# JCBrouwer/maua-style

Measured on AMD Instinct MI355X. Metric: optimizer iterations/sec at 1024x1024 VGG-19, higher is better.
Workload: dtype f32 (fp16x3 split-precision MFMA, fp32 accumulate)

## Files before the change

maua-style_amd/csrc/conv_x3w.hip:

```cpp
#include <stdlib.h>

#include <type_traits>

#include "conv_host.hpp"
#include "fp16x3.hpp"

namespace maua {

constexpr int XW_COT = 64;
constexpr int XW_ROWS = 8, XW_PR = 10, XW_PC = 34;
constexpr int XW_NPOS = XW_PR * XW_PC;
constexpr int XW_NPOS_PAD = 344;
constexpr int XW_PLANE = XW_NPOS_PAD * 16;
constexpr int XW_PATCH_BYTES = 4 * XW_PLANE;
constexpr int XW_W_BYTES = 9 * 2 * 2 * XW_COT * 16;
constexpr int XW_ITEMS = 2 * XW_NPOS;

__global__ void pack_x3w_kernel(const float* __restrict__ w, unsigned short* __restrict__ bank, int cout, int cin, int backward,
                                float w_scale) {
    const int CO = backward ? cin : cout;
    const int CI = backward ? cout : cin;
    const int nchunk = (CI + 15) / 16, ntile = (CO + XW_COT - 1) / XW_COT;
    const int64_t total = (int64_t)nchunk * ntile * 9 * 2 * XW_COT * 8;
    for (int64_t e = (int64_t)blockIdx.x * blockDim.x + threadIdx.x; e < total; e += (int64_t)gridDim.x * blockDim.x) {
        int64_t r = e;
        const int ch = (int)(r % 8);
        r /= 8;
        const int co = (int)(r % XW_COT);
        r /= XW_COT;
        const int oct = (int)(r % 2);
        r /= 2;
        const int tap = (int)(r % 9);
        r /= 9;
        const int tile = (int)(r % ntile);
        const int chunk = (int)(r / ntile);
        const int o = tile * XW_COT + co, i = chunk * 16 + oct * 8 + ch;
        float v = 0.f;
        if (o < CO && i < CI) {
            if (!backward) v = w[((int64_t)o * cin + i) * 9 + tap];
            else v = w[((int64_t)i * cin + o) * 9 + (8 - tap)];
        }
        v *= w_scale;
        const _Float16 h = (_Float16)v;
        const _Float16 l = (_Float16)(v - (float)h);
        const int64_t base = ((int64_t)chunk * ntile + tile) * (XW_W_BYTES / 2);
        bank[base + ((((int64_t)tap * 2 + 0) * 2 + oct) * XW_COT + co) * 8 + ch] = __builtin_bit_cast(unsigned short, h);
        bank[base + ((((int64_t)tap * 2 + 1) * 2 + oct) * XW_COT + co) * 8 + ch] = __builtin_bit_cast(unsigned short, l);
    }
}

__device__ __forceinline__ void pack_dmat_x3w_body(const float* __restrict__ d, int C, unsigned short* __restrict__ bank,
                                                   float* __restrict__ inv) {
    __shared__ float wmax[16];
    const int tid = threadIdx.x;
    const int64_t total4 = (int64_t)C * C / 4;
    float m = 0.f;
    int64_t e = tid;
    for (; e + 7 * 1024 < total4; e += 8 * 1024) {
        float4 v[8];
#pragma unroll
        for (int u = 0; u < 8; ++u) v[u] = reinterpret_cast<const float4*>(d)[e + u * 1024];
#pragma unroll
        for (int u = 0; u < 8; ++u) m = fmaxf(fmaxf(m, fmaxf(fabsf(v[u].x), fabsf(v[u].y))), fmaxf(fabsf(v[u].z), fabsf(v[u].w)));
    }
    for (; e < total4; e += 1024) {
        const float4 v = reinterpret_cast<const float4*>(d)[e];
        m = fmaxf(fmaxf(m, fmaxf(fabsf(v.x), fabsf(v.y))), fmaxf(fabsf(v.z), fabsf(v.w)));
    }
    m = wave_max_nonneg(m);
    if ((tid & 63) == 0) wmax[tid >> 6] = m;
    __syncthreads();
    m = 0.f;
    for (int i = 0; i < 16; ++i) m = fmaxf(m, wmax[i]);
    float scale = 1.f;
    if (m > 0.f && m < 3.0e38f) {
        const int e = (int)((__builtin_bit_cast(unsigned, m) >> 23) & 0xffu) - 127;
        scale = __builtin_bit_cast(float, (unsigned)(127 + 5 - max(e, -100)) << 23);
    }
    if (tid == 0 && blockIdx.x == 0) inv[0] = 1.f / scale;
    const int nchunk = C / 16, ntile = (C + XW_COT - 1) / XW_COT;
    const int64_t groups = (int64_t)nchunk * ntile * 2 * XW_COT;
    for (int64_t e = (int64_t)blockIdx.x * 1024 + tid; e < groups; e += (int64_t)gridDim.x * 1024) {
        int64_t r = e;
        const int co = (int)(r % XW_COT);
        r /= XW_COT;
        const int oct = (int)(r % 2);
        r /= 2;
        const int tile = (int)(r % ntile);
        const int chunk = (int)(r / ntile);
        const int o = tile * XW_COT + co, i = chunk * 16 + oct * 8;
        u32x4 Hh = {0u, 0u, 0u, 0u}, Ll = {0u, 0u, 0u, 0u};
        if (o < C) {
            const float4 v0 = *reinterpret_cast<const float4*>(d + (int64_t)o * C + i);
            const float4 v1 = *reinterpret_cast<const float4*>(d + (int64_t)o * C + i + 4);
            const float v[8] = {v0.x * scale, v0.y * scale, v0.z * scale, v0.w * scale, v1.x * scale, v1.y * scale, v1.z * scale, v1.w * scale};
#pragma unroll
            for (int q = 0; q < 4; ++q) {
                const unsigned H = cvt_pk_f16(v[2 * q], v[2 * q + 1]);
                Hh[q] = H;
                Ll[q] = cvt_pk_f16(v[2 * q] - f16_lo(H), v[2 * q + 1] - f16_hi(H));
            }
        }
        unsigned char* base = reinterpret_cast<unsigned char*>(bank) + ((int64_t)chunk * ntile + tile) * 4096 + co * 16;
        *reinterpret_cast<u32x4*>(base + (0 * 2 + oct) * 1024) = Hh;
        *reinterpret_cast<u32x4*>(base + (1 * 2 + oct) * 1024) = Ll;
    }
}
__global__ void __launch_bounds__(1024) pack_dmat_x3w_kernel(const float* __restrict__ d, int C, unsigned short* __restrict__ bank,
                                                             float* __restrict__ inv) {
    pack_dmat_x3w_body(d, C, bank, inv);
}
struct DmatPackBatch {
    const float* d[4];
    unsigned short* bank[4];
    float* inv[4];
    int C[4];
};
__global__ void __launch_bounds__(1024) pack_dmat_x3w_batch_kernel(DmatPackBatch b) {
    pack_dmat_x3w_body(b.d[blockIdx.y], b.C[blockIdx.y], b.bank[blockIdx.y], b.inv[blockIdx.y]);
}

#ifdef XW_STAMP
#define XW_MARK(k)                                                                                          \
    do {                                                                                                    \
        if (lane == 0 && p.mask) {                                                                          \
            const unsigned long long t_ = __builtin_amdgcn_s_memtime();                                     \
            const_cast<float*>(p.mask)[((((int64_t)blockIdx.y * gridDim.x + blockIdx.x) * 4 + wave) * 64 + (ch - ch_begin)) * 8 + (k)] = \
                __builtin_bit_cast(float, (unsigned)t_);                                                    \
        }                                                                                                   \
    } while (0)
#else
#define XW_MARK(k) do {} while (0)
#endif
#ifdef XW_STAMP
#define XW_END_STAMP()                                                                                      \
    do {                                      \
        asm volatile("s_waitcnt vmcnt(0)" ::: "memory");                                                    \
        if (lane == 0 && p.mask)                                                                            \
            const_cast<float*>(p.mask)[((((int64_t)blockIdx.y * gridDim.x + blockIdx.x) * 4 + wave) * 64 + 63) * 8 + 6] = \
                __builtin_bit_cast(float, (unsigned)__builtin_amdgcn_s_memtime());                          \
    } while (0)
#else
#define XW_END_STAMP() do {} while (0)
#endif

__device__ __forceinline__ const ConvArgs* xw_kernel_arguments() {
#if defined(__HIP_DEVICE_COMPILE__)
    return (const ConvArgs*)__builtin_amdgcn_kernarg_segment_ptr();
#else
    return nullptr;
#endif
}

template <bool ACC, bool OM, bool POOL = false, bool UNPOOL = false>
__global__ void __launch_bounds__(256, 2) conv_x3w_kernel(ConvArgs p, float w_inv_scale) {
    __shared__ __attribute__((aligned(16))) unsigned char smem[XW_PATCH_BYTES + XW_W_BYTES + 32];
    unsigned char* Pl = smem;
    unsigned char* Wl = smem + XW_PATCH_BYTES;
    float* Ml = reinterpret_cast<float*>(smem + XW_PATCH_BYTES + XW_W_BYTES);

    const int tid = threadIdx.x;
    const int lane = tid & 63, wave = tid >> 6;
    const int j = lane & 31, half = lane >> 5;
    const int wv = __builtin_amdgcn_readfirstlane(wave);
    const int ksplit = p.ksplit > 1 ? p.ksplit : 1;
    const int n = blockIdx.z / ksplit, split = blockIdx.z - n * ksplit;
    const int ntile = gridDim.y;
    const int tiles_total = p.tiles_x * ((p.OH + XW_ROWS - 1) / XW_ROWS);
    const int per_xcd = (tiles_total + 7) >> 3;
    const int xcd = blockIdx.x & 7;
    const int slot = (int)((blockIdx.y * gridDim.x + blockIdx.x) >> 3);
    const int cotile = p.cot_inner ? slot % ntile : (int)blockIdx.y;
    const int tile = xcd * per_xcd + (p.cot_inner ? slot / ntile : (int)(blockIdx.x >> 3));
    const int co0 = cotile * XW_COT;
    const int in_plane = p.H * p.W;
    const int64_t out_plane = (int64_t)p.OH * p.OW;
    const int st_w = UNPOOL ? p.W >> 1 : p.W;
    const int st_plane = UNPOOL ? (p.H >> 1) * (p.W >> 1) : in_plane;
    const float* __restrict__ xin = p.x + (int64_t)n * p.Cin * st_plane;
    const unsigned char* __restrict__ xcodes = UNPOOL ? p.in_codes + (int64_t)n * p.Cin * st_plane : nullptr;
    const unsigned code_mask = (unsigned)p.in_code_mask;
    if (tile >= min((xcd + 1) * per_xcd, tiles_total)) return;
    const int x0 = (tile % p.tiles_x) * 32, y0 = (tile / p.tiles_x) * XW_ROWS;
    if (tid == 0) {
        reinterpret_cast<int*>(Ml)[5] = (n * ntile + cotile) * tiles_total + tile;
        reinterpret_cast<int*>(Ml)[6] = split;
    }

    unsigned voff[3], lds_w[3];
    unsigned vcode = 0x80000000u, inmask = 0;
    if constexpr (UNPOOL) {
        constexpr int PR = XW_ROWS / 2 + 2, PCW = 18;
        const int oct = tid >= PR * PCW ? 1 : 0;
        const int rem = tid - oct * PR * PCW;
        const int pr = rem / PCW, pc = rem - pr * PCW;
        const int ppy = ((y0 - p.pad) >> 1) + pr, ppx = ((x0 - p.pad) >> 1) + pc;
        const bool item = tid < 2 * PR * PCW;
        const bool ok = item && ppy >= 0 && ppy < (p.H >> 1) && ppx >= 0 && ppx < st_w;
        const int pidx = ppy * st_w + ppx;
        voff[0] = ok ? (unsigned)(oct * 8 * st_plane + pidx) * 4u : 0x80000000u;
        vcode = ok ? (unsigned)(oct * st_plane + pidx) * 8u : 0x80000000u;
        const int r0 = 2 * ppy - (y0 - p.pad), c0 = 2 * ppx - (x0 - p.pad);
#pragma unroll
        for (int q = 0; q < 4; ++q) {
            const int r = r0 + (q >> 1), c = c0 + (q & 1);
            if (item && r >= 0 && r < XW_ROWS + 2 && c >= 0 && c < XW_PC) inmask |= 1u << q;
        }
        lds_w[0] = (unsigned)(oct * XW_PLANE + (r0 * XW_PC + c0) * 16);
        voff[1] = voff[2] = 0x80000000u;
        lds_w[1] = lds_w[2] = 0;
    } else {
#pragma unroll
        for (int k = 0; k < 3; ++k) {
            const int idx = tid + 256 * k;
            const int oct = idx >= XW_NPOS ? 1 : 0;
            const int pos = idx - oct * XW_NPOS;
            const int r = pos / XW_PC, c = pos - r * XW_PC;
            const int iy = y0 + r - p.pad, ix = x0 + c - p.pad;
            const bool ok = idx < XW_ITEMS && iy >= 0 && iy < p.H && ix >= 0 && ix < p.W;
            voff[k] = ok ? (unsigned)(oct * 8 * in_plane + iy * p.W + ix) * 4u : 0x80000000u;
            lds_w[k] = (unsigned)(oct * XW_PLANE + pos * 16);
        }
    }
    const unsigned range = (unsigned)in_plane * 64u;
    const unsigned range_x = (unsigned)st_plane * 64u;
    constexpr int NI = UNPOOL ? 1 : 3;
    float rp[NI][8];
    u32x2 cd = {0u, 0u};
    unsigned sel2[4];
    u32x4 hl[3][2];
    const int nmain = p.Cin / 16;
    const int n2 = p.dbank ? p.Cout / 16 : 0;
    const float* __restrict__ fin = p.dbank ? p.omask + (int64_t)n * p.Cout * in_plane : nullptr;
    auto load_patch = [&](int ch) {
        asm volatile("" : "+s"(ch));
        const __amdgpu_buffer_rsrc_t rs = __builtin_amdgcn_make_buffer_rsrc(const_cast<float*>(xin + (int64_t)ch * 16 * st_plane), 0, range_x, 0x00020000);
        if constexpr (UNPOOL) {
            const __amdgpu_buffer_rsrc_t rc = __builtin_amdgcn_make_buffer_rsrc(const_cast<unsigned char*>(xcodes + (int64_t)ch * 16 * st_plane), 0,
                                                                                range_x >> 2, 0x00020000);
            cd = __builtin_amdgcn_raw_buffer_load_b64(rc, vcode, 0, 0);
        }
#pragma unroll
        for (int c = 0; c < 8; ++c)
#pragma unroll
            for (int k = 0; k < NI; ++k)
                rp[k][c] = __builtin_bit_cast(float, __builtin_amdgcn_raw_buffer_load_b32(rs, voff[k], c * st_plane * 4, 0));
    };
    auto publish_max = [&]() {
        if constexpr (UNPOOL) {
            const unsigned m2 = code_mask * 0x00010001u;
#pragma unroll
            for (int i = 0; i < 4; ++i) {
                sel2[i] = __builtin_amdgcn_perm(0u, cd[i >> 1], (i & 1) ? 0x0c030c02u : 0x0c010c00u) & m2;
                const unsigned s0 = sel2[i] & 0xffffu, s1 = sel2[i] >> 16;
                rp[0][2 * i] = ((inmask >> s0) & 1u) ? rp[0][2 * i] : 0.f;
                rp[0][2 * i + 1] = ((inmask >> s1) & 1u) ? rp[0][2 * i + 1] : 0.f;
            }
        }
        float m = 0.f;
#pragma unroll
        for (int k = 0; k < NI; ++k)
#pragma unroll
            for (int c = 0; c < 8; ++c) m = fmaxf(m, fabsf(rp[k][c]));
        m = wave_max_nonneg(m);
        if (lane == 0) Ml[UNPOOL ? wv : wave] = m;
    };
    float sx = 1.f;
    auto chunk_scale = [&]() {
        const float m = fmaxf(fmaxf(Ml[0], Ml[1]), fmaxf(Ml[2], Ml[3]));
        int e = (int)((__builtin_bit_cast(unsigned, m) >> 23) & 0xffu) - 127;
        e = m > 0.f ? max(e, -100) : 11;
        sx = __builtin_bit_cast(float, (unsigned)(127 + 11 - e) << 23);
        return __builtin_bit_cast(float, (unsigned)(127 + e - 11) << 23);
    };
    auto corner_of = [&](int q, int part, int i) {
        const unsigned t = sel2[i] ^ ((unsigned)q * 0x00010001u);
        const unsigned keep = ((t & 0xffffu) ? 0u : 0xffffu) | ((t >> 16) ? 0u : 0xffff0000u);
        return hl[2][part][i] & keep;
    };
    auto split_item = [&](int k) {
        if constexpr (UNPOOL) {
            if (k == 1) {
#pragma unroll
                for (int q = 0; q < 2; ++q)
#pragma unroll
                    for (int i = 0; i < 4; ++i) {
                        hl[q][0][i] = corner_of(q, 0, i);
                        hl[q][1][i] = corner_of(q, 1, i);
                    }
            }
            if (k > 0) return;
        }
        const int dst = UNPOOL ? 2 : k;
#pragma unroll
        for (int q = 0; q < 4; ++q) {
            const float v0 = rp[k][2 * q] * sx, v1 = rp[k][2 * q + 1] * sx;
            const unsigned H = cvt_pk_f16(v0, v1);
            const unsigned Lo = cvt_pk_f16(v0 - f16_lo(H), v1 - f16_hi(H));
            hl[dst][0][q] = H;
            hl[dst][1][q] = Lo;
        }
    };
    auto store_patch = [&]() {
        if constexpr (UNPOOL) {
#pragma unroll
            for (int q = 0; q < 4; ++q)
                if ((inmask >> q) & 1u) {
                    const unsigned dst = lds_w[0] + (unsigned)(((q >> 1) * XW_PC + (q & 1)) * 16);
                    u32x4 h, l;
                    if (q < 2) {
                        h = hl[q][0];
                        l = hl[q][1];
                    } else {
#pragma unroll
                        for (int i = 0; i < 4; ++i) {
                            h[i] = corner_of(q, 0, i);
                            l[i] = corner_of(q, 1, i);
                        }
                    }
                    *reinterpret_cast<u32x4*>(Pl + dst) = h;
                    *reinterpret_cast<u32x4*>(Pl + 2 * XW_PLANE + dst) = l;
                }
            return;
        }
#pragma unroll
        for (int k = 0; k < NI; ++k) {
            if (k == 2 && tid >= XW_ITEMS - 512) break;
            *reinterpret_cast<u32x4*>(Pl + lds_w[k]) = hl[k][0];
            *reinterpret_cast<u32x4*>(Pl + 2 * XW_PLANE + lds_w[k]) = hl[k][1];
        }
    };

    const unsigned char* __restrict__ bank = reinterpret_cast<const unsigned char*>(p.w6);
    const unsigned lane16 = lane * 16;
    auto dma_filters = [&](int ch, int first, int count) {
        const unsigned char* src = bank + ((int64_t)ch * ntile + cotile) * XW_W_BYTES;
#pragma unroll
        for (int i = 0; i < count; ++i) {
            const int q = first + wv + 4 * i;
            const unsigned char* g = src + q * 1024;
            const unsigned lds_dst = (unsigned)(size_t)(__attribute__((address_space(3))) unsigned char*)(Wl + q * 1024);
            unsigned keep;
            asm volatile("s_mov_b32 %0, m0\n\ts_mov_b32 m0, %2\n\ts_nop 0\n\tglobal_load_lds_dwordx4 %1, %3\n\ts_mov_b32 m0, %0"
                         : "=&s"(keep)
                         : "v"(lane16), "s"(__builtin_amdgcn_readfirstlane(lds_dst)), "s"(g)
                         : "memory");
        }
    };

    const unsigned char* __restrict__ dbank = reinterpret_cast<const unsigned char*>(p.dbank);
    const float d_inv_scale = p.dbank ? p.dinv[n] : 0.f;

    const int b_base = half * XW_PLANE + ((2 * wave) * XW_PC + j) * 16;
    const int a_base = half * 1024 + j * 16;

    f32x16 acc[2][2], master[2][2];
    {
        const bool with_bias = p.bias != nullptr && p.ksplit <= 1;
#pragma unroll
        for (int t = 0; t < 2; ++t)
#pragma unroll
            for (int r = 0; r < 16; ++r) {
                const int co = co0 + t * 32 + (r & 3) + 8 * (r >> 2) + 4 * half;
                float b0 = 0.f;
                if (with_bias) b0 = p.bias[min(co, p.Cout - 1)];
                master[t][0][r] = b0;
                master[t][1][r] = b0;
                acc[t][0][r] = 0.f;
                acc[t][1][r] = 0.f;
            }
    }

    typedef f16x8 AFrag[2];
    typedef f16x8 BFrag[2][2];
    auto load_a = [&](AFrag& a, int tap, int t) {
#pragma unroll
        for (int part = 0; part < 2; ++part)
            a[part] = *reinterpret_cast<const f16x8*>(Wl + a_base + (tap * 2 + part) * 2048 + t * 512);
    };
    auto load_b = [&](BFrag& b, int tap) {
        const int ky = tap / 3, kx = tap - 3 * ky;
#pragma unroll
        for (int row = 0; row < 2; ++row)
#pragma unroll
            for (int part = 0; part < 2; ++part)
                b[row][part] = *reinterpret_cast<const f16x8*>(Pl + b_base + part * 2 * XW_PLANE + ((row + ky) * XW_PC + kx) * 16);
    };
    auto mfma_half = [&](const AFrag& a, const BFrag& b, int t) {
#pragma unroll
        for (int row = 0; row < 2; ++row) {
            acc[t][row] = __builtin_amdgcn_mfma_f32_32x32x16_f16(a[1], b[row][0], acc[t][row], 0, 0, 0);
            acc[t][row] = __builtin_amdgcn_mfma_f32_32x32x16_f16(a[0], b[row][1], acc[t][row], 0, 0, 0);
            acc[t][row] = __builtin_amdgcn_mfma_f32_32x32x16_f16(a[0], b[row][0], acc[t][row], 0, 0, 0);
        }
    };
    AFrag a0, a1;
    BFrag bx, by;
#define XW_FENCE() __builtin_amdgcn_sched_barrier(0)
#define XW_TAP(TAP, BCUR, BNXT, HAS_NEXT, EXTRA0, EXTRA1) \
    do {                                                  \
        load_a(a1, TAP, 1);                               \
        if (HAS_NEXT) load_b(BNXT, (TAP) + 1);            \
        XW_FENCE();                                       \
        mfma_half(a0, BCUR, 0);                           \
        EXTRA0;                                           \
        XW_FENCE();                                       \
        if (HAS_NEXT) load_a(a0, (TAP) + 1, 0);           \
        XW_FENCE();                                       \
        mfma_half(a1, BCUR, 1);                           \
        EXTRA1;                                           \
        XW_FENCE();                                       \
    } while (0)

    const int nchunks_all = nmain + n2;
    const int cps = (nchunks_all + ksplit - 1) / ksplit;
    const int ch_begin = split * cps;
    const int nchunks = min(nchunks_all, ch_begin + cps);
    float inv_cur = 0.f, inv_next = 0.f;
    if (ch_begin < min(nchunks, nmain)) {
        dma_filters(ch_begin, 0, 9);
        load_patch(ch_begin);
        publish_max();
        asm volatile("s_waitcnt lgkmcnt(0)" ::: "memory");
        __builtin_amdgcn_s_barrier();
        inv_cur = chunk_scale() * w_inv_scale;
        inv_next = inv_cur;
#pragma unroll
        for (int k = 0; k < 3; ++k) split_item(k);
        store_patch();
        asm volatile("s_waitcnt vmcnt(0) lgkmcnt(0)" ::: "memory");
        __builtin_amdgcn_s_barrier();
    }

    if (p.stagger > 0) {
        const int tg_slot = (__builtin_amdgcn_s_getreg((4 - 1) << 11 | 16 << 6 | 4) & 1);
        const int flat = blockIdx.x + gridDim.x * (blockIdx.y + gridDim.y * blockIdx.z);
        if (tg_slot && flat < 512)
            for (int i = 0; i < p.stagger; ++i) __builtin_amdgcn_s_sleep(8);
    }

#ifdef XW_STAMP
    if (lane == 0 && p.mask) {
        float* d_ = const_cast<float*>(p.mask) + ((((int64_t)blockIdx.y * gridDim.x + blockIdx.x) * 4 + wave) * 64 + 63) * 8;
        d_[0] = __builtin_bit_cast(float, (unsigned)__builtin_amdgcn_s_getreg((32 - 1) << 11 | 0 << 6 | 4));
        d_[1] = __builtin_bit_cast(float, (unsigned)__builtin_amdgcn_s_memtime());
        d_[2] = __builtin_bit_cast(float, (unsigned)__builtin_amdgcn_s_memrealtime());
    }
#endif
    const int main_end = min(nchunks, nmain);
    const int d_begin = max(ch_begin, nmain);
    for (int ch = ch_begin; ch < main_end; ++ch) {
        const bool more = ch + 1 < main_end;
        XW_MARK(0);
        load_b(bx, 0);
        load_a(a0, 0, 0);
        if (more) load_patch(ch + 1);
        XW_FENCE();
        XW_TAP(0, bx, by, true, (void)0, (void)0);
        XW_TAP(1, by, bx, true, (void)0, (void)0);
        XW_TAP(2, bx, by, true, (void)0, (void)0);
        XW_TAP(3, by, bx, true, (void)0, (void)0);
        XW_TAP(4, bx, by, true, (void)0, if (more) publish_max());
        XW_MARK(1);
        asm volatile("s_waitcnt lgkmcnt(0)" ::: "memory");
        XW_MARK(2);
        __builtin_amdgcn_s_barrier();
        XW_MARK(3);
        if (more) {
            dma_filters(ch + 1, 0, 5);
            inv_next = chunk_scale() * w_inv_scale;
        }
        XW_FENCE();
        XW_TAP(5, by, bx, true, if (more) split_item(0), (void)0);
        XW_TAP(6, bx, by, true, if (more) split_item(1), (void)0);
        XW_TAP(7, by, bx, true, if (more) split_item(2), (void)0);
        XW_TAP(8, bx, by, false, (void)0, (void)0);
        XW_MARK(4);
        asm volatile("s_waitcnt lgkmcnt(0)" ::: "memory");
        __builtin_amdgcn_s_barrier();
        XW_MARK(5);
        if (more) {
            dma_filters(ch + 1, 20, 4);
            store_patch();
        }
#pragma unroll
        for (int t = 0; t < 2; ++t)
#pragma unroll
            for (int row = 0; row < 2; ++row)
#pragma unroll
                for (int r = 0; r < 16; ++r) {
                    master[t][row][r] = fmaf(acc[t][row][r], inv_cur, master[t][row][r]);
                    acc[t][row][r] = 0.f;
                }
        inv_cur = inv_next;
        XW_MARK(6);
        if (more) {
            asm volatile("s_waitcnt vmcnt(0) lgkmcnt(0)" ::: "memory");
            XW_MARK(7);
            __builtin_amdgcn_s_barrier();
        }
    }

#ifdef XW_STAMP
    if (lane == 0 && p.mask) {
        float* d_ = const_cast<float*>(p.mask) + ((((int64_t)blockIdx.y * gridDim.x + blockIdx.x) * 4 + wave) * 64 + 63) * 8;
        d_[5] = __builtin_bit_cast(float, (unsigned)__builtin_amdgcn_s_memtime());
    }
#endif
    [[maybe_unused]] unsigned fbits[2] = {0u, 0u};
    [[maybe_unused]] const bool mask_from_bits = OM && p.mask_bits != 0;
    if constexpr (!POOL) if (d_begin < nchunks) {
        unsigned voff_f[2];
#pragma unroll
        for (int row = 0; row < 2; ++row) {
            const int oy = y0 + 2 * wave + row, oxx = x0 + j;
            voff_f[row] = (oy < p.H && oxx < p.W) ? (unsigned)(half * 8 * in_plane + oy * p.W + oxx) * 4u : 0x80000000u;
        }
        struct DChunk {
            float f[2][8];
            u32x4 a[2][2];
        };
        auto request = [&](DChunk& d, int c2) {
            asm volatile("" : "+s"(c2));
            const __amdgpu_buffer_rsrc_t rs = __builtin_amdgcn_make_buffer_rsrc(const_cast<float*>(fin + (int64_t)c2 * 16 * in_plane), 0, range, 0x00020000);
#pragma unroll
            for (int c = 0; c < 8; ++c)
#pragma unroll
                for (int row = 0; row < 2; ++row)
                    d.f[row][c] = __builtin_bit_cast(float, __builtin_amdgcn_raw_buffer_load_b32(rs, voff_f[row], c * in_plane * 4, 0));
            const unsigned char* g = dbank + (((int64_t)n * n2 + c2) * ntile + cotile) * 4096 + half * 1024 + j * 16;
#pragma unroll
            for (int part = 0; part < 2; ++part)
#pragma unroll
                for (int t = 0; t < 2; ++t) d.a[part][t] = *reinterpret_cast<const u32x4*>(g + part * 2048 + t * 512);
        };
        const int c2_begin = d_begin - nmain, c2_end = nchunks - nmain;
        DChunk da, db;
        request(da, c2_begin);
        __builtin_amdgcn_s_barrier();
        auto multiply = [&](DChunk& d, int c2) {
            if constexpr (OM) {
                const unsigned k = (unsigned)(c2 - (co0 >> 4));
                if (mask_from_bits && k < 4u) {
#pragma unroll
                    for (int row = 0; row < 2; ++row) {
                        unsigned b8 = 0;
#pragma unroll
                        for (int c = 0; c < 8; ++c) b8 |= d.f[row][c] > 0.f ? 1u << c : 0u;
                        fbits[row] |= b8 << (8 * k);
                    }
                }
            }
            float m = 0.f;
#pragma unroll
            for (int row = 0; row < 2; ++row)
#pragma unroll
                for (int c = 0; c < 8; ++c) m = fmaxf(m, fabsf(d.f[row][c]));
            m = wave_max_nonneg(m);
            int e = (int)((__builtin_bit_cast(unsigned, m) >> 23) & 0xffu) - 127;
            e = m > 0.f ? max(e, -100) : 11;
            const float s = __builtin_bit_cast(float, (unsigned)(127 + 11 - e) << 23);
            const float inv = __builtin_bit_cast(float, (unsigned)(127 + e - 11) << 23) * d_inv_scale;
            BFrag b;
#pragma unroll
            for (int row = 0; row < 2; ++row) {
                u32x4 Hh, Ll;
#pragma unroll
                for (int q = 0; q < 4; ++q) {
                    const float v0 = d.f[row][2 * q] * s, v1 = d.f[row][2 * q + 1] * s;
                    const unsigned H = cvt_pk_f16(v0, v1);
                    Hh[q] = H;
                    Ll[q] = cvt_pk_f16(v0 - f16_lo(H), v1 - f16_hi(H));
                }
                b[row][0] = __builtin_bit_cast(f16x8, Hh);
                b[row][1] = __builtin_bit_cast(f16x8, Ll);
            }
#pragma unroll
            for (int t = 0; t < 2; ++t) {
                AFrag a;
                a[0] = __builtin_bit_cast(f16x8, d.a[0][t]);
                a[1] = __builtin_bit_cast(f16x8, d.a[1][t]);
                mfma_half(a, b, t);
            }
#pragma unroll
            for (int t = 0; t < 2; ++t)
#pragma unroll
                for (int row = 0; row < 2; ++row)
#pragma unroll
                    for (int q = 0; q < 16; ++q) {
                        master[t][row][q] = fmaf(acc[t][row][q], inv, master[t][row][q]);
                        acc[t][row][q] = 0.f;
                    }
        };
        for (int c2 = c2_begin; c2 < c2_end; c2 += 2) {
            if (c2 + 1 < c2_end) request(db, c2 + 1);
            multiply(da, c2);
            if (c2 + 1 < c2_end) {
                if (c2 + 2 < c2_end) request(da, c2 + 2);
                multiply(db, c2 + 1);
            }
        }
    }

#ifdef XW_STAMP
    if (lane == 0 && p.mask) {
        float* d_ = const_cast<float*>(p.mask) + ((((int64_t)blockIdx.y * gridDim.x + blockIdx.x) * 4 + wave) * 64 + 63) * 8;
        d_[3] = __builtin_bit_cast(float, (unsigned)__builtin_amdgcn_s_memtime());
        d_[4] = __builtin_bit_cast(float, (unsigned)__builtin_amdgcn_s_memrealtime());
    }
#endif
    bool final_sums = p.ksplit <= 1;
    const ConvArgs* kp = xw_kernel_arguments();
    asm volatile("" : "+s"(kp));
    if (kp->ksplit > 1 && kp->arrive != nullptr) {
        const int ksplit = kp->ksplit;
        const int unit = __builtin_amdgcn_readfirstlane(reinterpret_cast<const int*>(Ml)[5]);
        const int split = __builtin_amdgcn_readfirstlane(reinterpret_cast<const int*>(Ml)[6]);
        unsigned* const arrive = kp->arrive + unit;
        const float* const bias = kp->bias;
        constexpr unsigned SLAB = XW_COT * XW_ROWS * 32 * 4;
        const __amdgpu_buffer_rsrc_t srs = __builtin_amdgcn_make_buffer_rsrc(reinterpret_cast<unsigned char*>(kp->ws) + (int64_t)unit * ksplit * SLAB, 0,
                                                                            (unsigned)ksplit * SLAB, 0x00020000);
        const unsigned toff = (unsigned)tid * 16u;
#pragma unroll
        for (int q = 0; q < 16; ++q) {
            const f32x16& m = master[q >> 3][(q >> 2) & 1];
            const f32x4 v = {m[4 * (q & 3)], m[4 * (q & 3) + 1], m[4 * (q & 3) + 2], m[4 * (q & 3) + 3]};
            __builtin_amdgcn_raw_buffer_store_b128(__builtin_bit_cast(u32x4, v), srs, toff, (unsigned)split * SLAB + q * 4096u, 16);
        }
        asm volatile("s_waitcnt vmcnt(0)" ::: "memory");
        __builtin_amdgcn_s_barrier();
        unsigned* tick = reinterpret_cast<unsigned*>(Ml) + 4;
        if (tid == 0) *tick = __hip_atomic_fetch_add(arrive, 1u, __ATOMIC_RELAXED, __HIP_MEMORY_SCOPE_AGENT);
        asm volatile("s_waitcnt vmcnt(0) lgkmcnt(0)" ::: "memory");
        __builtin_amdgcn_s_barrier();
        if ((int)*tick != ksplit - 1) return;
        if (tid == 0) __hip_atomic_store(arrive, 0u, __ATOMIC_RELAXED, __HIP_MEMORY_SCOPE_AGENT);
#pragma unroll
        for (int t = 0; t < 2; ++t)
#pragma unroll
            for (int row = 0; row < 2; ++row)
#pragma unroll
                for (int r = 0; r < 16; ++r) acc[t][row][r] = 0.f;
        for (int k = 0; k < ksplit; ++k) {
            if (k == split) {
#pragma unroll
                for (int t = 0; t < 2; ++t)
#pragma unroll
                    for (int row = 0; row < 2; ++row) acc[t][row] += master[t][row];
            } else {
#pragma unroll
                for (int q0 = 0; q0 < 16; q0 += 8) {
                    u32x4 tq[8];
#pragma unroll
                    for (int q = 0; q < 8; ++q) tq[q] = __builtin_amdgcn_raw_buffer_load_b128(srs, toff, (unsigned)k * SLAB + (q0 + q) * 4096u, 16);
#pragma unroll
                    for (int q = 0; q < 8; ++q) {
                        const f32x4 v = __builtin_bit_cast(f32x4, tq[q]);
                        f32x16& a = acc[(q0 + q) >> 3][((q0 + q) >> 2) & 1];
#pragma unroll
                        for (int e = 0; e < 4; ++e) a[4 * ((q0 + q) & 3) + e] += v[e];
                    }
                }
            }
        }
#pragma unroll
        for (int t = 0; t < 2; ++t)
#pragma unroll
            for (int r = 0; r < 16; ++r) {
                const int co = co0 + t * 32 + (r & 3) + 8 * (r >> 2) + 4 * half;
                const float b0 = bias != nullptr ? bias[min(co, kp->Cout - 1)] : 0.f;
                master[t][0][r] = acc[t][0][r] + b0;
                master[t][1][r] = acc[t][1][r] + b0;
            }
        final_sums = true;
    }
    if constexpr (POOL) if (final_sums) {
        const int PW = p.OW >> 1;
        const int64_t pplane = (int64_t)(p.OH >> 1) * PW;
        float* __restrict__ py = p.y + (int64_t)n * p.Cout * pplane;
        unsigned char* __restrict__ pc = p.pool_codes + (int64_t)n * p.Cout * pplane;
        const int oy = y0 + 2 * wave, oxx = x0 + j;
        const bool store = (lane & 1) == 0 && oy + 1 < p.OH && oxx + 1 < p.OW;
        const int64_t ppix = (int64_t)(oy >> 1) * PW + (oxx >> 1);
#pragma unroll
        for (int t = 0; t < 2; ++t)
#pragma unroll
            for (int q = 0; q < 4; ++q) {
                const int cq = co0 + t * 32 + 8 * q + 4 * half;
                unsigned pk = 0;
#pragma unroll
                for (int i = 0; i < 4; ++i) {
                    const int r = 4 * q + i;
                    float a = master[t][0][r], c = master[t][1][r];
                    a = a > 0.f ? a : 0.f;
                    c = c > 0.f ? c : 0.f;
                    const float b = __builtin_bit_cast(float, __builtin_amdgcn_update_dpp(0, __builtin_bit_cast(int, a), 0x101, 0xf, 0xf, false));
                    const float d = __builtin_bit_cast(float, __builtin_amdgcn_update_dpp(0, __builtin_bit_cast(int, c), 0x101, 0xf, 0xf, false));
                    float m = a;
                    unsigned arg = 0;
                    if (b > m) { m = b; arg = 1; }
                    if (c > m) { m = c; arg = 2; }
                    if (d > m) { m = d; arg = 3; }
                    pk |= (arg | (m > 0.f ? 0u : 4u)) << (8 * i);
                    if (store && cq < p.Cout) py[(int64_t)(cq + i) * pplane + ppix] = m;
                }
                if (store && cq < p.Cout) *reinterpret_cast<unsigned*>(pc + ((int64_t)(cq >> 3) * pplane + ppix) * 8 + 4 * half) = pk;
            }
        return;
    }
    float* __restrict__ yout = p.y + (int64_t)n * p.Cout * out_plane;
    const float* __restrict__ om = p.omask ? p.omask + (int64_t)n * p.Cout * out_plane : nullptr;
    const int ox = x0 + j;
    auto store_rows = [&](auto reuse) {
        constexpr bool BITS = decltype(reuse)::value;
        [[maybe_unused]] unsigned ebits[2][2];
        if constexpr (BITS) {
#pragma unroll
            for (int row = 0; row < 2; ++row) {
                const unsigned other = (unsigned)__builtin_amdgcn_ds_bpermute((lane ^ 32) << 2, (int)fbits[row]);
                ebits[row][0] = (half ? other : fbits[row]) >> (4 * half);
                ebits[row][1] = (half ? fbits[row] : other) >> (4 * half);
            }
        }
#pragma unroll
        for (int row = 0; row < 2; ++row) {
            const int oy = y0 + 2 * wave + row;
            const bool pvalid = oy < p.OH && ox < p.OW;
            const int64_t opix = (int64_t)oy * p.OW + ox;
            if (!final_sums) {
                float* wsp = p.ws + (int64_t)blockIdx.z * p.Cout * out_plane;
#pragma unroll
                for (int t = 0; t < 2; ++t)
#pragma unroll
                    for (int r = 0; r < 16; ++r) {
                        const int co = co0 + t * 32 + (r & 3) + 8 * (r >> 2) + 4 * half;
                        if (pvalid && co < p.Cout) wsp[(int64_t)co * out_plane + opix] = master[t][row][r];
                    }
                continue;
            }
            if (!pvalid) continue;
            const bool full = co0 + XW_COT <= p.Cout;
            const int64_t lane_off = (int64_t)(co0 + 4 * half) * out_plane + opix;
            float* __restrict__ yl = yout + lane_off;
            const float* __restrict__ oml = OM ? om + lane_off : nullptr;
#pragma unroll
            for (int t = 0; t < 2; ++t) {
                float prev[16], msk[16];
#pragma unroll
                for (int r = 0; r < 16; ++r) {
                    const int cr = t * 32 + (r & 3) + 8 * (r >> 2);
                    const int64_t o = (full || co0 + cr + 4 * half < p.Cout) ? (int64_t)cr * out_plane : 0;
                    prev[r] = 0.f;
                    msk[r] = 1.f;
                    if constexpr (ACC) prev[r] = yl[o];
                    if constexpr (OM && !BITS) msk[r] = oml[o];
                }
                float outv[16];
#pragma unroll
                for (int r = 0; r < 16; ++r) {
                    float v = master[t][row][r];
                    v += prev[r];
                    if (p.relu) v = v > 0.f ? v : 0.f;
                    bool keep = msk[r] > 0.f;
                    if constexpr (BITS) keep = ((ebits[row][(r >> 2) & 1] >> (8 * (2 * t + (r >> 3)) + (r & 3))) & 1u) != 0;
                    outv[r] = keep ? v : 0.f;
                }
                if (full) {
#pragma unroll
                    for (int r = 0; r < 16; ++r) yl[(int64_t)(t * 32 + (r & 3) + 8 * (r >> 2)) * out_plane] = outv[r];
                } else {
#pragma unroll
                    for (int r = 0; r < 16; ++r) {
                        const int cr = t * 32 + (r & 3) + 8 * (r >> 2);
                        if (co0 + cr + 4 * half < p.Cout) yl[(int64_t)cr * out_plane] = outv[r];
                    }
                }
            }
        }
    };
    if constexpr (OM) {
        if (mask_from_bits) {
            store_rows(std::true_type{});
            XW_END_STAMP();
            return;
        }
    }
    store_rows(std::false_type{});
    XW_END_STAMP();
}

static constexpr SplitModel XW_SPLIT = {.rows = XW_ROWS, .cot = XW_COT, .chunk = 16, .partial_chunk = false, .slots = 512,
                                             .no_split_wgs = 2048, .min_chunks = 4, .chunks_per_split = 2, .us_per_chunk = 4.0,
                                             .prologue_chunks = 1.0, .forced = "x3w_ks", .finish_in_launch = true};

bool conv_x3w_supports(const ConvArgs& a) {
    return a.Cin % 16 == 0 && (int64_t)a.H * a.W <= (1ll << 25) && a.pad >= 0 && a.pad <= 2;
}

#ifdef XW_STAMP
static float* g_xw_stamp = nullptr;
extern "C" void maua_xw_set_stamp_buffer(float* buf) { g_xw_stamp = buf; }
#endif

int conv_x3w_launch(const ConvArgs& a, int n, float w_scale, hipStream_t stream) {
    ConvArgs p = a;
#ifdef XW_STAMP
    p.mask = g_xw_stamp;
#endif
    p.tiles_x = (a.OW + 31) / 32;
    p.cot_inner = tuning("cot_inner", 0) != 0 ? 1 : 0;
    const int64_t tiles = conv_tiles(a, XW_ROWS);
    const int ks = a.ws ? choose_split(XW_SPLIT, a) : 1;
    p.ksplit = ks;
    const int64_t cot = (a.Cout + XW_COT - 1) / XW_COT, per_xcd = (tiles + 7) / 8;
    dim3 grid((unsigned)(per_xcd * 8), (unsigned)cot, (unsigned)(n * ks));
    const bool whole = ks == 1 || finish_in_launch(XW_SPLIT, a, n, ks);
    if (!whole) p.arrive = nullptr;
    const bool acc = whole && a.accumulate != 0, om = whole && a.omask != nullptr;
    const float w_inv = 1.f / w_scale;
    {
        p.stagger = (int)tuning("x3w_stagger", 7);
    }
    p.mask_bits = (ks == 1 && a.dbank && om && tuning("gram_mask_reuse", 1) != 0) ? 1 : 0;
    if (a.pool_codes && whole) hipLaunchKernelGGL((conv_x3w_kernel<false, false, true>), grid, dim3(256), 0, stream, p, w_inv);
    else if (a.in_codes && om) hipLaunchKernelGGL((conv_x3w_kernel<false, true, false, true>), grid, dim3(256), 0, stream, p, w_inv);
    else if (a.in_codes) hipLaunchKernelGGL((conv_x3w_kernel<false, false, false, true>), grid, dim3(256), 0, stream, p, w_inv);
    else if (acc && om) hipLaunchKernelGGL((conv_x3w_kernel<true, true>), grid, dim3(256), 0, stream, p, w_inv);
    else if (acc) hipLaunchKernelGGL((conv_x3w_kernel<true, false>), grid, dim3(256), 0, stream, p, w_inv);
    else if (om) hipLaunchKernelGGL((conv_x3w_kernel<false, true>), grid, dim3(256), 0, stream, p, w_inv);
    else hipLaunchKernelGGL((conv_x3w_kernel<false, false>), grid, dim3(256), 0, stream, p, w_inv);
    int rc = check_launch("conv_x3w_kernel");
    if (rc || whole) return rc;
    return a.pool_codes ? conv_splitk_finish_pool(a, n, ks, stream) : conv_splitk_finish(a, n, ks, stream);
}

}

using namespace maua;

extern "C" {

size_t maua_conv_x3w_bank_bytes(int cout_produced, int cin_consumed) {
    return bank_bytes(cout_produced, cin_consumed, 16, XW_COT, XW_W_BYTES);
}

int maua_conv_pack_filters_x3w(const float* w_oihw, void* bank_fwd, void* bank_bwd, int cout, int cin, float w_scale,
                               maua_stream_t stream) {
    MAUA_REQUIRE(pack_args_ok(w_oihw, bank_fwd, bank_bwd, cout, cin) && w_scale > 0.f, MAUA_E_INVAL, "conv_pack_filters_x3w: bad args");
    return pack_two_banks(bank_fwd, bank_bwd, "pack_x3w_kernel", [&](unsigned short* bank, int backward) {
        hipLaunchKernelGGL(pack_x3w_kernel, dim3(1024), dim3(256), 0, (hipStream_t)stream, w_oihw, bank, cout, cin, backward, w_scale);
    });
}

size_t maua_conv_x3w_dmat_bank_bytes(int c) {
    if (c <= 0 || c % 16 != 0 || c > (1 << 14)) return 0;
    return (size_t)(c / 16) * ((c + XW_COT - 1) / XW_COT) * 4096;
}

int maua_conv_pack_dmat_x3w(const float* dmat, int c, void* bank, float* inv_scale_out, maua_stream_t stream) {
    MAUA_REQUIRE(dmat && bank && inv_scale_out && c > 0 && c % 16 == 0 && c <= (1 << 14), MAUA_E_INVAL,
                 "conv_pack_dmat_x3w: needs a C x C matrix with C %% 16 == 0");
    const int64_t groups = (int64_t)(c / 16) * ((c + XW_COT - 1) / XW_COT) * 2 * XW_COT;
    hipLaunchKernelGGL(pack_dmat_x3w_kernel, dim3((unsigned)((groups + 4095) / 4096)), dim3(1024), 0, (hipStream_t)stream, dmat, c,
                       (unsigned short*)bank, inv_scale_out);
    return check_launch("pack_dmat_x3w_kernel");
}

int maua_conv_pack_dmat_x3w_batch(int count, const float* const* dmats, const int* cs, void* const* banks, float* const* inv_scales_out,
                                  maua_stream_t stream) {
    MAUA_REQUIRE(count > 0 && count <= 4 && dmats && cs && banks && inv_scales_out, MAUA_E_INVAL, "conv_pack_dmat_x3w_batch: bad args (at most 4 layers)");
    DmatPackBatch b{};
    int64_t most = 0;
    for (int i = 0; i < count; ++i) {
        MAUA_REQUIRE(dmats[i] && banks[i] && inv_scales_out[i] && cs[i] > 0 && cs[i] % 16 == 0 && cs[i] <= (1 << 14), MAUA_E_INVAL,
                     "conv_pack_dmat_x3w_batch: layer %d needs a C x C matrix with C %% 16 == 0", i);
        b.d[i] = dmats[i];
        b.bank[i] = (unsigned short*)banks[i];
        b.inv[i] = inv_scales_out[i];
        b.C[i] = cs[i];
        const int64_t groups = (int64_t)(cs[i] / 16) * ((cs[i] + XW_COT - 1) / XW_COT) * 2 * XW_COT;
        most = groups > most ? groups : most;
    }
    hipLaunchKernelGGL(pack_dmat_x3w_batch_kernel, dim3((unsigned)((most + 4095) / 4096), (unsigned)count), dim3(1024), 0, (hipStream_t)stream, b);
    return check_launch("pack_dmat_x3w_batch_kernel");
}

int maua_conv_x3w_supported(int cin, int h, int w, int pad) {
    ConvArgs a;
    return conv_geometry(a, 1, cin, h, w, 1, 3, pad) != CONV_SHAPE_BAD_DIMS && conv_x3w_supports(a) ? 1 : 0;
}

size_t maua_conv_x3w_workspace_bytes(int n, int cin, int h, int w, int cout, int pad) {
    return query_workspace_bytes(XW_SPLIT, n, cin, h, w, cout, pad);
}

static int conv3x3_x3w_entry(const float* x, const void* bank, float w_scale, const float* bias, const float* out_relu_mask, float* y,
                             int n, int cin, int h, int w, int cout, int pad, int relu, int accumulate, const void* dbank,
                             const float* dinv, void* workspace, size_t workspace_bytes, maua_stream_t stream,
                             const unsigned char* in_codes = nullptr, int in_code_mask = 0) {
    MAUA_REQUIRE(x && bank && y && w_scale > 0.f, MAUA_E_INVAL, "conv3x3_x3w: bad args");
    ConvArgs a;
    const ConvShape shape = conv_geometry(a, n, cin, h, w, cout, 3, pad);
    MAUA_REQUIRE(shape != CONV_SHAPE_BAD_DIMS && pad <= 2, MAUA_E_INVAL, "conv3x3_x3w: bad dims");
    MAUA_REQUIRE(shape == CONV_SHAPE_OK, MAUA_E_UNSUPPORTED, "conv3x3_x3w: input smaller than the filter");
    a.x = x;
    a.w6 = bank;
    a.bias = bias;
    a.omask = out_relu_mask;
    a.y = y;
    a.relu = relu;
    a.accumulate = accumulate;
    MAUA_REQUIRE(conv_x3w_supports(a), MAUA_E_UNSUPPORTED, "conv3x3_x3w: needs cin %% 16 == 0 and a plane of at most 2^25 pixels");
    if (dbank) {
        MAUA_REQUIRE(dinv && out_relu_mask, MAUA_E_INVAL, "conv3x3_x3w_gram: needs the feature map and the bank's inverse scale");
        MAUA_REQUIRE(cout % 16 == 0 && a.OH == h && a.OW == w, MAUA_E_UNSUPPORTED,
                     "conv3x3_x3w_gram: needs cout %% 16 == 0 and an output plane of the input's size");
        a.dbank = dbank;
        a.dinv = dinv;
    }
    if (in_codes) {
        MAUA_REQUIRE(h >= 2 && w >= 2 && !accumulate, MAUA_E_UNSUPPORTED, "conv3x3_x3w_unpool: needs an input plane of 2 x 2 and more, no accumulation");
        a.in_codes = in_codes;
        a.in_code_mask = in_code_mask;
    }
    accept_workspace(a, workspace, workspace_bytes, true, XW_SPLIT, n);
    return conv_x3w_launch(a, n, w_scale, (hipStream_t)stream);
}

int maua_conv3x3_x3w(const float* x, const void* bank, float w_scale, const float* bias, const float* out_relu_mask, float* y,
                     int n, int cin, int h, int w, int cout, int pad, int relu, int accumulate, void* workspace,
                     size_t workspace_bytes, maua_stream_t stream) {
    return conv3x3_x3w_entry(x, bank, w_scale, bias, out_relu_mask, y, n, cin, h, w, cout, pad, relu, accumulate, nullptr, nullptr,
                             workspace, workspace_bytes, stream);
}

int maua_conv_x3w_split(int n, int cin, int h, int w, int cout, int pad) {
    return query_split(XW_SPLIT, n, cin, h, w, cout, pad);
}

int maua_conv3x3_x3w_relu_pool(const float* x, const void* bank, float w_scale, const float* bias, float* pooled,
                               unsigned char* codes, int n, int cin, int h, int w, int cout, int pad, void* workspace,
                               size_t workspace_bytes, maua_stream_t stream) {
    MAUA_REQUIRE(x && bank && pooled && codes && w_scale > 0.f, MAUA_E_INVAL, "conv3x3_x3w_relu_pool: bad args");
    ConvArgs a;
    MAUA_REQUIRE(conv_geometry(a, n, cin, h, w, cout, 3, pad) != CONV_SHAPE_BAD_DIMS && pad <= 2, MAUA_E_INVAL, "conv3x3_x3w_relu_pool: bad dims");
    a.x = x;
    a.w6 = bank;
    a.bias = bias;
    a.y = pooled;
    a.pool_codes = codes;
    a.relu = 1;
    MAUA_REQUIRE(a.OH >= 2 && a.OW >= 2 && cout % 8 == 0 && conv_x3w_supports(a), MAUA_E_UNSUPPORTED,
                 "conv3x3_x3w_relu_pool: needs an output plane of 2 x 2 and more, cin %% 16 == 0, cout %% 8 == 0");
    accept_workspace(a, workspace, workspace_bytes, true, XW_SPLIT, n);
    return conv_x3w_launch(a, n, w_scale, (hipStream_t)stream);
}

int maua_conv3x3_x3w_gram(const float* x, const void* bank, float w_scale, const float* feature_map, const void* dmat_bank,
                          const float* dmat_inv_scale, float* y, int n, int cin, int h, int w, int cout, int pad, int accumulate,
                          void* workspace, size_t workspace_bytes, maua_stream_t stream) {
    MAUA_REQUIRE(dmat_bank, MAUA_E_INVAL, "conv3x3_x3w_gram: null bank");
    return conv3x3_x3w_entry(x, bank, w_scale, nullptr, feature_map, y, n, cin, h, w, cout, pad, 0, accumulate, dmat_bank,
                             dmat_inv_scale, workspace, workspace_bytes, stream);
}

int maua_conv3x3_x3w_unpool(const float* pooled_x, const unsigned char* codes, int honour_relu_bit, const void* bank, float w_scale,
                            const float* out_relu_mask, const void* dmat_bank, const float* dmat_inv_scale, float* y, int n, int cin,
                            int h, int w, int cout, int pad, void* workspace, size_t workspace_bytes, maua_stream_t stream) {
    MAUA_REQUIRE(codes, MAUA_E_INVAL, "conv3x3_x3w_unpool: null decision bytes");
    return conv3x3_x3w_entry(pooled_x, bank, w_scale, nullptr, out_relu_mask, y, n, cin, h, w, cout, pad, 0, 0, dmat_bank, dmat_inv_scale,
                             workspace, workspace_bytes, stream, codes, honour_relu_bit ? 7 : 3);
}

}
```

Measured before the change: 201.7.

## Process delta chunks in pairs with shared exponent and interleaved prefetch

Restructures the secondary (delta) chunk loop to handle two 16-channel chunks per step. The two chunks share one wave-wide max reduction and one exponent-scale computation, and the master accumulation fold runs once per pair instead of once per chunk. Loads for the next pair are issued between MFMA calls, and out-of-range prefetches are clamped to a zero-range buffer descriptor. Sharing the scale across two chunks can slightly reduce split-precision accuracy when their magnitudes differ, and holding two chunks at once raises register pressure.

```diff
diff --git a/maua-style_amd/csrc/conv_x3w.hip b/maua-style_amd/csrc/conv_x3w.hip
--- a/maua-style_amd/csrc/conv_x3w.hip
+++ b/maua-style_amd/csrc/conv_x3w.hip
@@ -516,71 +516,93 @@
             const int oy = y0 + 2 * wave + row, oxx = x0 + j;
             voff_f[row] = (oy < p.H && oxx < p.W) ? (unsigned)(half * 8 * in_plane + oy * p.W + oxx) * 4u : 0x80000000u;
         }
-        struct DChunk {
-            float f[2][8];
-            u32x4 a[2][2];
-        };
-        auto request = [&](DChunk& d, int c2) {
-            asm volatile("" : "+s"(c2));
-            const __amdgpu_buffer_rsrc_t rs = __builtin_amdgcn_make_buffer_rsrc(const_cast<float*>(fin + (int64_t)c2 * 16 * in_plane), 0, range, 0x00020000);
-#pragma unroll
-            for (int c = 0; c < 8; ++c)
-#pragma unroll
-                for (int row = 0; row < 2; ++row)
-                    d.f[row][c] = __builtin_bit_cast(float, __builtin_amdgcn_raw_buffer_load_b32(rs, voff_f[row], c * in_plane * 4, 0));
-            const unsigned char* g = dbank + (((int64_t)n * n2 + c2) * ntile + cotile) * 4096 + half * 1024 + j * 16;
-#pragma unroll
-            for (int part = 0; part < 2; ++part)
-#pragma unroll
-                for (int t = 0; t < 2; ++t) d.a[part][t] = *reinterpret_cast<const u32x4*>(g + part * 2048 + t * 512);
+        struct DPair {
+            float f[2][2][8];
+            u32x4 a[2][2][2];
         };
         const int c2_begin = d_begin - nmain, c2_end = nchunks - nmain;
-        DChunk da, db;
-        request(da, c2_begin);
+        auto request_f = [&](DPair& d, int k, int c2) {
+            asm volatile("" : "+s"(c2));
+            const __amdgpu_buffer_rsrc_t rs = __builtin_amdgcn_make_buffer_rsrc(const_cast<float*>(fin + (int64_t)min(c2, c2_end - 1) * 16 * in_plane), 0,
+                                                                                c2 < c2_end ? range : 0u, 0x00020000);
+#pragma unroll
+            for (int c = 0; c < 8; ++c)
+#pragma unroll
+                for (int row = 0; row < 2; ++row)
+                    d.f[k][row][c] = __builtin_bit_cast(float, __builtin_amdgcn_raw_buffer_load_b32(rs, voff_f[row], c * in_plane * 4, 0));
+        };
+        auto request_a = [&](DPair& d, int k, int c2) {
+            asm volatile("" : "+s"(c2));
+            const unsigned char* g = dbank + (((int64_t)n * n2 + min(c2, c2_end - 1)) * ntile + cotile) * 4096 + half * 1024 + j * 16;
+#pragma unroll
+            for (int part = 0; part < 2; ++part)
+#pragma unroll
+                for (int t = 0; t < 2; ++t) d.a[k][part][t] = *reinterpret_cast<const u32x4*>(g + part * 2048 + t * 512);
+        };
+        DPair dp;
+#pragma unroll
+        for (int k = 0; k < 2; ++k) {
+            request_f(dp, k, c2_begin + k);
+            request_a(dp, k, c2_begin + k);
+        }
         __builtin_amdgcn_s_barrier();
-        auto multiply = [&](DChunk& d, int c2) {
+        auto multiply = [&](auto count, int c2) {
+            constexpr int NC = decltype(count)::value;
             if constexpr (OM) {
-                const unsigned k = (unsigned)(c2 - (co0 >> 4));
-                if (mask_from_bits && k < 4u) {
-#pragma unroll
-                    for (int row = 0; row < 2; ++row) {
-                        unsigned b8 = 0;
-#pragma unroll
-                        for (int c = 0; c < 8; ++c) b8 |= d.f[row][c] > 0.f ? 1u << c : 0u;
-                        fbits[row] |= b8 << (8 * k);
+#pragma unroll
+                for (int ck = 0; ck < NC; ++ck) {
+                    const unsigned k = (unsigned)(c2 + ck - (co0 >> 4));
+                    if (mask_from_bits && k < 4u) {
+#pragma unroll
+                        for (int row = 0; row < 2; ++row) {
+                            unsigned b8 = 0;
+#pragma unroll
+                            for (int c = 0; c < 8; ++c) b8 |= dp.f[ck][row][c] > 0.f ? 1u << c : 0u;
+                            fbits[row] |= b8 << (8 * k);
+                        }
                     }
                 }
             }
             float m = 0.f;
 #pragma unroll
-            for (int row = 0; row < 2; ++row)
-#pragma unroll
-                for (int c = 0; c < 8; ++c) m = fmaxf(m, fabsf(d.f[row][c]));
+            for (int ck = 0; ck < NC; ++ck)
+#pragma unroll
+                for (int row = 0; row < 2; ++row)
+#pragma unroll
+                    for (int c = 0; c < 8; ++c) m = fmaxf(m, fabsf(dp.f[ck][row][c]));
             m = wave_max_nonneg(m);
             int e = (int)((__builtin_bit_cast(unsigned, m) >> 23) & 0xffu) - 127;
             e = m > 0.f ? max(e, -100) : 11;
             const float s = __builtin_bit_cast(float, (unsigned)(127 + 11 - e) << 23);
             const float inv = __builtin_bit_cast(float, (unsigned)(127 + e - 11) << 23) * d_inv_scale;
-            BFrag b;
-#pragma unroll
-            for (int row = 0; row < 2; ++row) {
-                u32x4 Hh, Ll;
-#pragma unroll
-                for (int q = 0; q < 4; ++q) {
-                    const float v0 = d.f[row][2 * q] * s, v1 = d.f[row][2 * q + 1] * s;
-                    const unsigned H = cvt_pk_f16(v0, v1);
-                    Hh[q] = H;
-                    Ll[q] = cvt_pk_f16(v0 - f16_lo(H), v1 - f16_hi(H));
+            BFrag b[NC];
+#pragma unroll
+            for (int ck = 0; ck < NC; ++ck)
+#pragma unroll
+                for (int row = 0; row < 2; ++row) {
+                    u32x4 Hh, Ll;
+#pragma unroll
+                    for (int q = 0; q < 4; ++q) {
+                        const float v0 = dp.f[ck][row][2 * q], v1 = dp.f[ck][row][2 * q + 1];
+                        const unsigned H = cvt_pk_f16(v0 * s, v1 * s);
+                        Hh[q] = H;
+                        Ll[q] = cvt_pk_f16(fmaf(v0, s, -f16_lo(H)), fmaf(v1, s, -f16_hi(H)));
+                    }
+                    b[ck][row][0] = __builtin_bit_cast(f16x8, Hh);
+                    b[ck][row][1] = __builtin_bit_cast(f16x8, Ll);
                 }
-                b[row][0] = __builtin_bit_cast(f16x8, Hh);
-                b[row][1] = __builtin_bit_cast(f16x8, Ll);
-            }
-#pragma unroll
-            for (int t = 0; t < 2; ++t) {
-                AFrag a;
-                a[0] = __builtin_bit_cast(f16x8, d.a[0][t]);
-                a[1] = __builtin_bit_cast(f16x8, d.a[1][t]);
-                mfma_half(a, b, t);
+#pragma unroll
+            for (int ck = 0; ck < NC; ++ck) {
+                AFrag af[2];
+#pragma unroll
+                for (int t = 0; t < 2; ++t) {
+                    af[t][0] = __builtin_bit_cast(f16x8, dp.a[ck][0][t]);
+                    af[t][1] = __builtin_bit_cast(f16x8, dp.a[ck][1][t]);
+                }
+                if constexpr (NC == 2) request_f(dp, ck, c2 + 2 + ck);
+#pragma unroll
+                for (int t = 0; t < 2; ++t) mfma_half(af[t], b[ck], t);
+                if constexpr (NC == 2) request_a(dp, ck, c2 + 2 + ck);
             }
 #pragma unroll
             for (int t = 0; t < 2; ++t)
@@ -592,14 +614,9 @@
                         acc[t][row][q] = 0.f;
                     }
         };
-        for (int c2 = c2_begin; c2 < c2_end; c2 += 2) {
-            if (c2 + 1 < c2_end) request(db, c2 + 1);
-            multiply(da, c2);
-            if (c2 + 1 < c2_end) {
-                if (c2 + 2 < c2_end) request(da, c2 + 2);
-                multiply(db, c2 + 1);
-            }
-        }
+        int c2 = c2_begin;
+        for (; c2 + 1 < c2_end; c2 += 2) multiply(std::integral_constant<int, 2>{}, c2);
+        if (c2 < c2_end) multiply(std::integral_constant<int, 1>{}, c2);
     }
 
 #ifdef XW_STAMP
```

Result: no change. 201.9 (median of 6 runs) (+0.1%).
